# LeoIV/polyaxon

Measured on AMD Instinct MI355X. Metric: HPO trials/hour (whole node) + wall-clock-to-target, ResNet-50 Hyperband sweep, higher is better.
Workload: dtype bf16

## Files before the change

polyaxon_amd/csrc/bn_kernels.hip:

```cpp
#include <hip/hip_runtime.h>

#include "handoff.h"
#include <stdint.h>

#define PLX_API extern "C" __attribute__((visibility("default")))

namespace {

constexpr int kBlock = 256;

struct alignas(16) bf16x8 {
  uint16_t v[8];
};

__device__ __forceinline__ float bf2f(uint16_t b) { return __uint_as_float(((uint32_t)b) << 16); }

__device__ __forceinline__ uint16_t f2bf(float f) {
  return __builtin_bit_cast(uint16_t, (__bf16)f);
}

__device__ __forceinline__ void load8(const bf16x8* p, float* f) {
  const bf16x8 v = *p;
#pragma unroll
  for (int k = 0; k < 8; ++k) f[k] = bf2f(v.v[k]);
// ... 465 lines not shown
        ra[k] += g2;
        rc[k] = fmaf(g2, (x2[k] - mu2[k]) * is2[k], rc[k]);
      }
    }
    float o[8];
#pragma unroll
    for (int k = 0; k < 8; ++k) o[k] = fmaf(A[k], g[k], fmaf(B[k], xv[k], D[k]));
    store8(dx + i, o);
  }
  if constexpr (rp) {
  __shared__ float red[kBlock * 16];
#pragma unroll
  for (int k = 0; k < 8; ++k) {
    red[threadIdx.x * 16 + k] = ra[k];
    red[threadIdx.x * 16 + 8 + k] = rc[k];
  }
  __syncthreads();
  if ((int)threadIdx.x < G) {
    for (int j = 1; j < kBlock / G; ++j) {
      const float* o = red + (j * G + threadIdx.x) * 16;
#pragma unroll
      for (int k = 0; k < 8; ++k) {
        ra[k] += o[k];
        rc[k] += o[8 + k];
      }
    }
    float* pa = rb.part + (int64_t)blockIdx.x * C + cg * 8;
    float* pc = rb.part + ((int64_t)gridDim.x + blockIdx.x) * C + cg * 8;
#pragma unroll
    for (int k = 0; k < 8; ++k) {
      pa[k] = ra[k];
      pc[k] = rc[k];
    }
  }
  }
}

struct Plan {
  int G, Gb, gy, nblk, S;
  int64_t rows_per_block;
};

inline bool plan_for(int64_t M, int C, Plan* p) {
  if (C <= 0 || (C & 7)) return false;
  const int G = C / 8;
  if (G & (G - 1)) return false;
  p->G = G;
  p->Gb = G < kBlock ? G : kBlock;
  p->gy = G / p->Gb;
  const int R = kBlock / p->Gb;
  const int64_t cap = (2048 + p->gy - 1) / p->gy;
  int64_t want = (M + 16 * R - 1) / (16 * R);
  if (want > cap) want = cap;
  if (want < 1) want = 1;
  int64_t rpb = (M + want - 1) / want;
  rpb = (rpb + R - 1) / R * R;
  p->rows_per_block = rpb;
  p->nblk = (int)((M + rpb - 1) / rpb);
  p->S = (p->nblk + kRowsPerSplit - 1) / kRowsPerSplit;
  return true;
}

inline int apply_grid(int64_t n_vec, int G) {
  int64_t g = (n_vec + kBlock - 1) / kBlock;
  if (g > 4096) g = 4096;
  if (g < 1) g = 1;
  const int64_t mult = G > kBlock ? G / kBlock : 1;
  g = (g + mult - 1) / mult * mult;
  return (int)g;
}

inline void launch_dx(hipStream_t stream, int64_t n_vec, int G, const void* x, const uint8_t* mask, const void* dy,
                      void* dx, void* dres, const float* coef, int relu, const ResBn& rb) {
  const dim3 grid(apply_grid(n_vec, G));
  auto k = rb.part == nullptr ? (relu ? bn_bwd_dx_kernel<false, true> : bn_bwd_dx_kernel<false, false>)
           : rb.mask != nullptr ? (relu ? bn_bwd_dx_kernel<true, true, true> : bn_bwd_dx_kernel<true, false, true>)
                                : (relu ? bn_bwd_dx_kernel<true, true> : bn_bwd_dx_kernel<true, false>);
  hipLaunchKernelGGL(k, grid, dim3(kBlock), 0, stream, (const bf16x8*)x, mask, (const bf16x8*)dy, (bf16x8*)dx,
                     (bf16x8*)dres, coef, n_vec, G, relu, rb);
}

inline void launch_apply(hipStream_t stream, int64_t n_vec, int G, const void* x, const void* res, void* y,
                         const float* scale, const float* bias, int relu, uint8_t* mask, const float* rsb) {
  auto k = res != nullptr ? (relu ? bn_apply_kernel<true, true> : bn_apply_kernel<true, false>)
                          : (relu ? bn_apply_kernel<false, true> : bn_apply_kernel<false, false>);
  hipLaunchKernelGGL(k, dim3(apply_grid(n_vec, G)), dim3(kBlock), 0, stream, (const bf16x8*)x, (const bf16x8*)res,
                     (bf16x8*)y, scale, bias, n_vec, G, mask, rsb);
}

inline void reduce_finalize_fwd(hipStream_t stream, const float* part, int nblk, float* l2, unsigned* cnt,
                                const FwdFin& f) {
  const int C = f.C, S = (nblk + kRowsPerSplit - 1) / kRowsPerSplit;
  if (cnt != nullptr) {
    hipLaunchKernelGGL(bn_fwd_reduce_finalize_kernel<kFinNT>, dim3((C + 63) / 64, S), dim3(kFinNT), 0, stream, part, nblk, l2, S,
                       cnt, f);
    return;
  }
  hipLaunchKernelGGL(bn_partial_reduce_kernel<kFinNT>,
                     dim3((C + 63) / 64, S, 2), dim3(kFinNT), 0, stream, part, nblk, C, l2, S);
  hipLaunchKernelGGL(bn_fwd_finalize_kernel<kFinNT>, dim3((C + 63) / 64),
                     dim3(kFinNT), 0, stream, l2, l2 + (int64_t)S * C, S,
                     f.x_row0, C, f.M, f.gamma, f.beta, f.eps, f.momentum, f.running_mean, f.running_var, f.save_mean,
                     f.save_invstd, f.scale, f.bias);
}

inline void reduce_finalize_bwd(hipStream_t stream, const float* part, int nblk, float* l2, unsigned* cnt,
                                const BwdFin& f) {
  const int C = f.C, S = (nblk + kRowsPerSplit - 1) / kRowsPerSplit;
  if (cnt != nullptr) {
    hipLaunchKernelGGL(bn_bwd_reduce_finalize_kernel<kFinNT>, dim3((C + 63) / 64, S), dim3(kFinNT), 0, stream, part, nblk, l2, S,
                       cnt, f);
    return;
  }
  hipLaunchKernelGGL(bn_partial_reduce_kernel<kFinNT>,
                     dim3((C + 63) / 64, S, 2), dim3(kFinNT), 0, stream, part, nblk, C, l2, S);
  hipLaunchKernelGGL(bn_bwd_finalize_kernel<kFinNT>, dim3((C + 63) / 64),
                     dim3(kFinNT), 0, stream, l2, l2 + (int64_t)S * C, S, C,
                     f.M, f.gamma, f.mean, f.invstd, f.dgamma, f.dbeta, f.coef, f.accumulate);
}

struct alignas(8) u8x8 {
  uint8_t v[8];
};

__global__ __launch_bounds__(256) void stem_apply_pool_kernel(const bf16x8* __restrict__ x,
                                                              const float* __restrict__ sb, bf16x8* __restrict__ y,
                                                              u8x8* __restrict__ idx, int N, int H, int W, int G,
                                                              int OH, int OW) {
  const unsigned j = blockIdx.x * 256u + threadIdx.x;
  if (j >= (unsigned)(OW * G)) return;
  const unsigned g = j % (unsigned)G, ow = j / (unsigned)G;
  const int C = G * 8;
  float a[8], b[8];
#pragma unroll
  for (int k = 0; k < 8; ++k) {
    a[k] = sb[g * 8 + k];
    b[k] = sb[C + g * 8 + k];
  }
  for (int row = blockIdx.y; row < N * OH; row += gridDim.y) {
    const int n = row / OH, oh = row - n * OH;
    float best[8];
    uint8_t arg[8];
#pragma unroll
    for (int k = 0; k < 8; ++k) {
      best[k] = -INFINITY;
      arg[k] = 255;
    }
    uint4 q[9];
    bool ok[9];
#pragma unroll
    for (int kh = 0; kh < 3; ++kh) {
      const int ih = oh * 2 - 1 + kh;
      const int ihc = ih < 0 ? 0 : (ih >= H ? H - 1 : ih);
#pragma unroll
      for (int kw = 0; kw < 3; ++kw) {
        const int iw = (int)ow * 2 - 1 + kw;
        const int iwc = iw < 0 ? 0 : (iw >= W ? W - 1 : iw);
        ok[kh * 3 + kw] = ih >= 0 && ih < H && iw >= 0 && iw < W;
        q[kh * 3 + kw] = *(const uint4*)(x + ((size_t)(n * H + ihc) * W + iwc) * G + g);
      }
    }
#pragma unroll
    for (int t9 = 0; t9 < 9; ++t9) {
      const uint32_t qw[4] = {q[t9].x, q[t9].y, q[t9].z, q[t9].w};
#pragma unroll
      for (int k = 0; k < 8; ++k) {
        const float xk = __uint_as_float((k & 1) ? (qw[k >> 1] & 0xffff0000u) : (qw[k >> 1] << 16));
        const float f = (float)(__bf16)fmaxf(fmaf(xk, a[k], b[k]), 0.f);
        if (ok[t9] && (f > best[k] || arg[k] == 255)) {
          best[k] = f;
          arg[k] = (uint8_t)t9;
        }
      }
    }
    bf16x8 o;
    u8x8 m;
#pragma unroll
    for (int k = 0; k < 8; ++k) {
      o.v[k] = f2bf(best[k]);
      m.v[k] = arg[k];
    }
    const size_t t = (size_t)row * OW * G + j;
    y[t] = o;
    idx[t] = m;
  }
}

__device__ __forceinline__ int stem_cover(int i, int O, int* o, int* k) {
  int n = 0;
  if (i & 1) {
    if ((i + 1) >> 1 < O) { o[n] = (i + 1) >> 1; k[n++] = 0; }
    o[n] = (i - 1) >> 1; k[n++] = 2;
  } else if ((i >> 1) < O) {
    o[n] = i >> 1; k[n++] = 1;
  }
  return n;
}

template <bool DX>
__global__ __launch_bounds__(256) void stem_pool_bn_bwd_kernel(const bf16x8* __restrict__ dy, const u8x8* __restrict__ idx,
                                                               const bf16x8* __restrict__ x, const float* __restrict__ sb,
                                                               const float* __restrict__ mean,
                                                               const float* __restrict__ invstd,
                                                               const float* __restrict__ coef, bf16x8* __restrict__ dx,
                                                               float* __restrict__ part, int N, int H, int W, int G,
                                                               int OH, int OW) {
  const int QH = (H + 1) / 2, QW = (W + 1) / 2;
  const unsigned j0 = blockIdx.x * 256u + threadIdx.x;
  const bool active = j0 < (unsigned)(QW * G);
  const unsigned j = active ? j0 : 0u;
  const unsigned g = j % (unsigned)G;
  const int qb = (int)(j / (unsigned)G);
  const int C = G * 8;
  float a[8], b[8], c1[8], c2[8], c3[8], s1[8], s2[8];
#pragma unroll
  for (int k = 0; k < 8; ++k) {
    a[k] = sb[g * 8 + k];
    b[k] = sb[C + g * 8 + k];
    if constexpr (DX) {
      c1[k] = coef[g * 8 + k];
      c2[k] = coef[C + g * 8 + k];
      c3[k] = coef[2 * C + g * 8 + k];
    } else {
      c1[k] = mean[g * 8 + k];
      c2[k] = invstd[g * 8 + k];
      c3[k] = 0.f;
    }
    s1[k] = s2[k] = 0.f;
  }
  for (int row = blockIdx.y; active && row < N * QH; row += gridDim.y) {
    const int n = row / QH, qa = row - n * QH;
    uint2 am[4];
    uint4 d[4], xq[4];
    bool wv[4], pv[4];
#pragma unroll
    for (int p = 0; p < 2; ++p)
#pragma unroll
      for (int q = 0; q < 2; ++q) {
        const int w4 = p * 2 + q, oh = qa + p, ow = qb + q;
        wv[w4] = oh < OH && ow < OW;
        const size_t off = ((size_t)(n * OH + (oh < OH ? oh : OH - 1)) * OW + (ow < OW ? ow : OW - 1)) * G + g;
        am[w4] = *(const uint2*)(idx + off);
        d[w4] = *(const uint4*)(dy + off);
        if (!wv[w4]) am[w4] = make_uint2(0xffffffffu, 0xffffffffu);
        const int ih = 2 * qa + p, iw = 2 * qb + q;
        pv[w4] = ih < H && iw < W;
        xq[w4] = *(const uint4*)(x + ((size_t)(n * H + (ih < H ? ih : H - 1)) * W + (iw < W ? iw : W - 1)) * G + g);
      }
#pragma unroll
    for (int di = 0; di < 2; ++di)
#pragma unroll
      for (int dj = 0; dj < 2; ++dj) {
        const int e = di * 2 + dj;
        const uint32_t xw[4] = {xq[e].x, xq[e].y, xq[e].z, xq[e].w};
        float o[8];
#pragma unroll
        for (int k = 0; k < 8; ++k) {
          float acc = 0.f;
#pragma unroll
          for (int p = 0; p < 2; ++p)
#pragma unroll
            for (int q = 0; q < 2; ++q) {
              const int kh = di + 1 - 2 * p, kw = dj + 1 - 2 * q;
              if (kh < 0 || kw < 0) continue;
              const int w4 = p * 2 + q;
              const uint32_t ab = (k < 4 ? am[w4].x : am[w4].y) >> (8 * (k & 3)) & 0xffu;
              const uint32_t dw = (k >> 1) == 0 ? d[w4].x : (k >> 1) == 1 ? d[w4].y : (k >> 1) == 2 ? d[w4].z : d[w4].w;
              const float dv = __uint_as_float((k & 1) ? (dw & 0xffff0000u) : (dw << 16));
              acc += ab == (uint32_t)(kh * 3 + kw) ? dv : 0.f;
            }
          const float xf = __uint_as_float((k & 1) ? (xw[k >> 1] & 0xffff0000u) : (xw[k >> 1] << 16));
          const float dz = (pv[e] && fmaf(xf, a[k], b[k]) > 0.f) ? (float)(__bf16)acc : 0.f;
          if constexpr (DX) {
            o[k] = fmaf(c1[k], dz, fmaf(c2[k], xf, c3[k]));
          } else {
            s1[k] += dz;
            s2[k] = fmaf(dz, (xf - c1[k]) * c2[k], s2[k]);
          }
        }
        if constexpr (DX) {
          if (pv[e]) store8(dx + ((size_t)(n * H + 2 * qa + di) * W + 2 * qb + dj) * G + g, o);
        }
      }
  }
  if constexpr (!DX) {
    __shared__ float red[256 * 17];
#pragma unroll
    for (int k = 0; k < 8; ++k) {
      red[threadIdx.x * 17 + k] = s1[k];
      red[threadIdx.x * 17 + 8 + k] = s2[k];
    }
    __syncthreads();
    const int nb = gridDim.x * gridDim.y, blk = blockIdx.y * gridDim.x + blockIdx.x;
    for (int e = threadIdx.x; e < G * 16; e += 256) {
      const int gg = e % G, v = e / G;
      float sum = 0.f;
      for (int r = gg; r < 256; r += G) sum += red[r * 17 + v];
      const int c = gg * 8 + (v & 7);
      part[((int64_t)(v < 8 ? 0 : nb) + blk) * C + c] = sum;
    }
  }
}

constexpr int g_stem_bwd_cap = 4096;

inline dim3 stem_bwd_grid(int N, int H, int W, int G, bool dx) {
  const int rows = N * ((H + 1) / 2), cap = dx ? 65535 : g_stem_bwd_cap;
  return dim3((((W + 1) / 2) * G + 255) / 256, rows < cap ? rows : cap);
}

}

PLX_API int64_t plx_bn_workspace(int64_t M, int C) {
  Plan p;
  if (!plan_for(M, C, &p)) return -1;
  return 2 * (int64_t)(p.nblk + p.S) * C;
}

PLX_API int plx_bn_forward(const void* x, const void* res, void* y, int64_t M, int C, const float* gamma,
                           const float* beta, float eps, float momentum, float* running_mean, float* running_var,
                           float* save_mean, float* save_invstd, float* scale_bias ,
                           float* partials , uint8_t* mask ,
                           int relu, const float* res_sb ,
                           unsigned* counters ,
                           hipStream_t stream) {
  Plan p;
  if (!plan_for(M, C, &p) || M < 1) return 1;
  float* psum = partials;
  float* psq = partials + (int64_t)p.nblk * C;
  hipLaunchKernelGGL(bn_stats_kernel, dim3(p.nblk, p.gy), dim3(kBlock), 0, stream, (const bf16x8*)x, M, p.G, p.Gb,
                     p.rows_per_block, psum, psq);
  float* l2 = partials + 2 * (int64_t)p.nblk * C;
  reduce_finalize_fwd(stream, partials, p.nblk, l2, counters,
                      FwdFin{(const uint16_t*)x, C, M, gamma, beta, eps, momentum, running_mean, running_var,
                             save_mean, save_invstd, scale_bias, scale_bias + C});
  const int64_t n_vec = M * p.G;
  if (y != nullptr)
    launch_apply(stream, n_vec, p.G, x, res, y, scale_bias, scale_bias + C, relu, relu ? mask : nullptr, res_sb);
  return (int)hipGetLastError();
}

PLX_API int64_t plx_bn_l2_workspace(int nblk, int C) {
  return 2 * (int64_t)((nblk + kRowsPerSplit - 1) / kRowsPerSplit) * C;
}

PLX_API int plx_bn_forward_from_partials(const void* x, const void* res, void* y, int64_t M, int C,
                                         const float* gamma, const float* beta, float eps, float momentum,
                                         float* running_mean, float* running_var, float* save_mean,
                                         float* save_invstd, float* scale_bias, const float* partials, int nblk,
                                         float* l2, uint8_t* mask, int relu, const float* res_sb,
                                         unsigned* counters, hipStream_t stream) {
  Plan p;
  if (!plan_for(M, C, &p) || M < 1 || nblk < 1) return 1;
  reduce_finalize_fwd(stream, partials, nblk, l2, counters,
                      FwdFin{nullptr, C, M, gamma, beta, eps, momentum, running_mean, running_var, save_mean,
                             save_invstd, scale_bias, scale_bias + C});
  const int64_t n_vec = M * p.G;
  if (y != nullptr)
    launch_apply(stream, n_vec, p.G, x, res, y, scale_bias, scale_bias + C, relu, relu ? mask : nullptr, res_sb);
  return (int)hipGetLastError();
}

PLX_API int plx_bn_apply(const void* x, const void* res, void* y, int64_t M, int C, const float* scale_bias, int relu,
                         hipStream_t stream) {
  Plan p;
  if (!plan_for(M, C, &p)) return 1;
  const int64_t n_vec = M * p.G;
  launch_apply(stream, n_vec, p.G, x, res, y, scale_bias, scale_bias + C, relu, nullptr, nullptr);
  return (int)hipGetLastError();
}

PLX_API int plx_bn_apply_res_relu(const void* x, const void* res, void* y, int64_t M, int C, const float* scale_bias,
                                  uint8_t* mask, const float* res_sb, hipStream_t stream) {
  Plan p;
  if (!plan_for(M, C, &p) || M < 1 || res == nullptr || mask == nullptr) return 1;
  launch_apply(stream, M * p.G, p.G, x, res, y, scale_bias, scale_bias + C, 1, mask, res_sb);
  return (int)hipGetLastError();
}

PLX_API int plx_bn_dx_blocks(int64_t M, int C) {
  Plan p;
  if (!plan_for(M, C, &p)) return -1;
  return apply_grid(M * p.G, p.G);
}

PLX_API int plx_bn_backward(const void* x, const uint8_t* mask, const void* dy, void* dx, void* dres, int64_t M, int C,
                            const float* gamma, const float* save_mean, const float* save_invstd, float* dgamma,
                            float* dbeta, float* coef , float* partials , int relu,
                            int accumulate, const ResBn* resbn , unsigned* counters,
                            hipStream_t stream) {
  Plan p;
  if (!plan_for(M, C, &p) || M < 1 || (relu && mask == nullptr)) return 1;
  if (resbn != nullptr && (dres == nullptr || resbn->part == nullptr)) return 1;
  const ResBn rb = resbn != nullptr ? *resbn : ResBn{};
  float* pa = partials;
  float* pb = partials + (int64_t)p.nblk * C;
  hipLaunchKernelGGL(relu ? bn_bwd_reduce_kernel<true> : bn_bwd_reduce_kernel<false>, dim3(p.nblk, p.gy), dim3(kBlock), 0, stream, (const bf16x8*)x,
                     mask, (const bf16x8*)dy, M, p.G, p.Gb, p.rows_per_block, save_mean, save_invstd,
                     relu, pa, pb);
  float* l2 = partials + 2 * (int64_t)p.nblk * C;
  reduce_finalize_bwd(stream, partials, p.nblk, l2, counters,
                      BwdFin{C, M, gamma, save_mean, save_invstd, dgamma, dbeta, coef, accumulate});
  const int64_t n_vec = M * p.G;
  launch_dx(stream, n_vec, p.G, x, mask, dy, dx, dres, coef, relu, rb);
  return (int)hipGetLastError();
}

PLX_API int plx_bn_backward_from_partials(const void* x, const uint8_t* mask, const void* dy, void* dx, void* dres,
                                          int64_t M, int C, const float* gamma, const float* save_mean,
                                          const float* save_invstd, float* dgamma, float* dbeta, float* coef,
                                          const float* partials, int nblk, float* l2, int relu, int accumulate,
                                          const ResBn* resbn, unsigned* counters, hipStream_t stream) {
  Plan p;
  if (!plan_for(M, C, &p) || M < 1 || nblk < 1 || (relu && mask == nullptr)) return 1;
  if (resbn != nullptr && (dres == nullptr || resbn->part == nullptr)) return 1;
  const ResBn rb = resbn != nullptr ? *resbn : ResBn{};
  reduce_finalize_bwd(stream, partials, nblk, l2, counters,
                      BwdFin{C, M, gamma, save_mean, save_invstd, dgamma, dbeta, coef, accumulate});
  const int64_t n_vec = M * p.G;
  launch_dx(stream, n_vec, p.G, x, mask, dy, dx, dres, coef, relu, rb);
  return (int)hipGetLastError();
}

PLX_API int plx_bn_backward_coef(const void* x, const uint8_t* mask, const void* dy, int64_t M, int C,
                                 const float* gamma, const float* save_mean, const float* save_invstd, float* dgamma,
                                 float* dbeta, float* coef, float* partials, int relu, int accumulate,
                                 unsigned* counters, hipStream_t stream) {
  Plan p;
  if (!plan_for(M, C, &p) || M < 1 || (relu && mask == nullptr)) return 1;
  float* pa = partials;
  float* pb = partials + (int64_t)p.nblk * C;
  hipLaunchKernelGGL(relu ? bn_bwd_reduce_kernel<true> : bn_bwd_reduce_kernel<false>, dim3(p.nblk, p.gy), dim3(kBlock), 0, stream, (const bf16x8*)x,
                     mask, (const bf16x8*)dy, M, p.G, p.Gb, p.rows_per_block, save_mean, save_invstd,
                     relu, pa, pb);
  reduce_finalize_bwd(stream, partials, p.nblk, partials + 2 * (int64_t)p.nblk * C, counters,
                      BwdFin{C, M, gamma, save_mean, save_invstd, dgamma, dbeta, coef, accumulate});
  return (int)hipGetLastError();
}

PLX_API int plx_bn_backward_coef_from_partials(int64_t M, int C, const float* gamma, const float* save_mean,
                                               const float* save_invstd, float* dgamma, float* dbeta, float* coef,
                                               const float* partials, int nblk, float* l2, int accumulate,
                                               unsigned* counters, hipStream_t stream) {
  Plan p;
  if (!plan_for(M, C, &p) || M < 1 || nblk < 1) return 1;
  reduce_finalize_bwd(stream, partials, nblk, l2, counters,
                      BwdFin{C, M, gamma, save_mean, save_invstd, dgamma, dbeta, coef, accumulate});
  return (int)hipGetLastError();
}

PLX_API int plx_stem_bn_pool_forward(const void* x, void* y, void* idx, int N, int H, int W, int C, const float* gamma,
                                     const float* beta, float eps, float momentum, float* running_mean,
                                     float* running_var, float* save_mean, float* save_invstd, float* scale_bias,
                                     float* partials, const float* ext_part, int ext_nblk, unsigned* counters,
                                     hipStream_t stream) {
  const int G = C / 8;
  if (N <= 0 || H <= 0 || W <= 0 || C % 8 || G > 256 || 256 % G) return 1;
  const int rc = ext_part != nullptr
                     ? plx_bn_forward_from_partials(x, nullptr, nullptr, (int64_t)N * H * W, C, gamma, beta, eps,
                                                    momentum, running_mean, running_var, save_mean, save_invstd,
                                                    scale_bias, ext_part, ext_nblk, partials, nullptr, 1, nullptr,
                                                    counters, stream)
                     : plx_bn_forward(x, nullptr, nullptr, (int64_t)N * H * W, C, gamma, beta, eps, momentum,
                                      running_mean, running_var, save_mean, save_invstd, scale_bias, partials, nullptr,
                                      1, nullptr, counters, stream);
  if (rc) return rc;
  const int OH = (H - 1) / 2 + 1, OW = (W - 1) / 2 + 1;
  const int rows = N * OH;
  hipLaunchKernelGGL(stem_apply_pool_kernel, dim3((OW * G + 255) / 256, rows < 65535 ? rows : 65535), dim3(256), 0,
                     stream, (const bf16x8*)x, scale_bias, (bf16x8*)y, (u8x8*)idx, N, H, W, G, OH, OW);
  return (int)hipGetLastError();
}


PLX_API int64_t plx_stem_bn_pool_bwd_workspace(int N, int H, int W, int C) {
  const dim3 g = stem_bwd_grid(N, H, W, C / 8, false);
  const int64_t nblk = (int64_t)g.x * g.y;
  return 2 * (nblk + (nblk + kRowsPerSplit - 1) / kRowsPerSplit) * C;
}

PLX_API int plx_stem_bn_pool_backward(const void* dy, const void* idx, const void* x, void* dx, int N, int H, int W,
                                      int C, const float* gamma, const float* save_mean, const float* save_invstd,
                                      const float* scale_bias, float* dgamma, float* dbeta, float* coef,
                                      float* workspace, int accumulate, unsigned* counters, hipStream_t stream) {
  const int G = C / 8;
  if (N <= 0 || H <= 0 || W <= 0 || C % 8 || G > 256 || 256 % G) return 1;
  const int OH = (H - 1) / 2 + 1, OW = (W - 1) / 2 + 1;
  const dim3 grid = stem_bwd_grid(N, H, W, G, false), grid_dx = stem_bwd_grid(N, H, W, G, true);
  const int nblk = grid.x * grid.y;
  hipLaunchKernelGGL(stem_pool_bn_bwd_kernel<false>, grid, dim3(256), 0, stream, (const bf16x8*)dy, (const u8x8*)idx,
                     (const bf16x8*)x, scale_bias, save_mean, save_invstd, (const float*)nullptr, (bf16x8*)nullptr,
                     workspace, N, H, W, G, OH, OW);
  reduce_finalize_bwd(stream, workspace, nblk, workspace + 2 * (int64_t)nblk * C, counters,
                      BwdFin{C, (int64_t)N * H * W, gamma, save_mean, save_invstd, dgamma, dbeta, coef, accumulate});
  hipLaunchKernelGGL(stem_pool_bn_bwd_kernel<true>, grid_dx, dim3(256), 0, stream, (const bf16x8*)dy, (const u8x8*)idx,
                     (const bf16x8*)x, scale_bias, save_mean, save_invstd, coef, (bf16x8*)dx, (float*)nullptr, N, H,
                     W, G, OH, OW);
  return (int)hipGetLastError();
}
```

polyaxon_amd/ops/_native.py:

```python
from __future__ import annotations

import ctypes
import hashlib
import os
import shutil
import subprocess
import threading
from pathlib import Path
from typing import Dict, Iterable, List, Optional

PKG_DIR = Path(__file__).resolve().parent.parent
CSRC = PKG_DIR / "csrc"
OUT = PKG_DIR / "_native"
ARCH = os.environ.get("PLX_OFFLOAD_ARCH", "gfx950")
ROCM = Path(os.environ.get("ROCM_PATH", "/opt/rocm"))

LIBRARIES: Dict[str, dict] = {
    "plx_train": {"sources": ["train_kernels.hip"], "kind": "hip", "link": []},
    "plx_polytune": {"sources": ["polytune_kernels.hip"], "kind": "hip", "link": []},
    "plx_bn": {"sources": ["bn_kernels.hip"], "kind": "hip", "link": []},
    "plx_procmon": {"sources": ["procmon.cpp"], "kind": "cpp", "link": ["-lpthread"]},
    "plx_gp": {"sources": ["gp_kernels.hip", "gp_chol.hip"], "kind": "hip", "link": []},
    "plx_rms": {"sources": ["rmsnorm.hip"], "kind": "hip", "link": []},
    "plx_conv": {"sources": ["conv_gemm.hip"], "kind": "hip", "link": []},
    "plx_pool": {"sources": ["pool_kernels.hip"], "kind": "hip", "link": []},
    "plx_lm": {"sources": ["lm_kernels.hip"], "kind": "hip", "link": []},
    "plx_gemm": {"sources": ["gemm256.hip"], "kind": "hip", "link": []},
    "plx_attn": {"sources": ["attn_kernels.hip"], "kind": "hip", "link": []},
    "plx_rccl": {"sources": ["rccl_comm.cpp"], "kind": "hip_host", "link": ["-lrccl", "-pthread"]},
}

_lock = threading.Lock()
_loaded: Dict[str, ctypes.CDLL] = {}


def _register(name: str, sources: List[str], kind: str, link: Optional[List[str]] = None) -> None:
    LIBRARIES[name] = {"sources": sources, "kind": kind, "link": list(link or [])}


def lib_path(name: str) -> Path:
    return OUT / f"lib{name}.so"


def _digest(sources: Iterable[Path], flags: List[str]) -> str:
    h = hashlib.sha256()
    for s in sources:
        h.update(s.read_bytes())
    for hdr in sorted(CSRC.glob("*.h")):
        h.update(hdr.read_bytes())
    h.update(" ".join(flags).encode())
    return h.hexdigest()[:16]


def _flags(kind: str) -> List[str]:
    common = ["-O3", "-std=c++17", "-shared", "-fPIC", "-Wall", "-Wno-unused-function", f"-I{CSRC}"]
    if kind == "hip":
        fences = ["-DPLX_HANDOFF_FENCES=1"] if os.environ.get("PLX_HANDOFF_FENCES") == "1" else []
        return common + [f"--offload-arch={ARCH}", "-munsafe-fp-atomics"] + fences
    if kind == "hip_host":
        return common + [f"-I{ROCM / 'include'}", "-D__HIP_PLATFORM_AMD__"]
    return common


def build(name: str, force: bool = False, verbose: bool = False) -> Path:
    spec = LIBRARIES[name]
    srcs = [CSRC / s for s in spec["sources"]]
    flags = _flags(spec["kind"])
    out = lib_path(name)
    stamp = out.with_suffix(".so.sha")
    digest = _digest(srcs, flags + spec["link"])
    if not force and out.exists() and stamp.exists() and stamp.read_text().strip() == digest:
        return out
    OUT.mkdir(parents=True, exist_ok=True)
    if spec["kind"] in ("hip", "hip_host"):
        cc = shutil.which("hipcc") or str(ROCM / "bin" / "hipcc")
    else:
        cc = shutil.which("g++") or "g++"
    link = list(spec["link"])
    if spec["kind"] == "hip_host":
        link = [f"-L{ROCM / 'lib'}", f"-Wl,-rpath,{ROCM / 'lib'}"] + link + ["-lamdhip64"]
    tmp = out.with_suffix(f".so.tmp{os.getpid()}")
    cmd = [cc, *flags, *map(str, srcs), "-o", str(tmp), *link]
    if verbose:
        print(" ".join(cmd))
    proc = subprocess.run(cmd, capture_output=True, text=True)
    if proc.returncode != 0:
        raise RuntimeError(f"native build of {name} failed:\n{' '.join(cmd)}\n{proc.stderr[-6000:]}")
    os.replace(tmp, out)
    stamp.write_text(digest)
    return out


def _stale(name: str) -> bool:
    spec = LIBRARIES[name]
    stamp = lib_path(name).with_suffix(".so.sha")
    if not stamp.exists():
        return False
    try:
        digest = _digest([CSRC / s for s in spec["sources"]], _flags(spec["kind"]) + spec["link"])
    except OSError:
        return False
    return stamp.read_text().strip() != digest


def build_all(force: bool = False, verbose: bool = False) -> List[Path]:
    return [build(n, force=force, verbose=verbose) for n in LIBRARIES]


def available(name: str) -> bool:
    return lib_path(name).exists()


_SIZES: Dict[tuple, int] = {}


_COUNTERS: Dict[tuple, object] = {}


def capturing() -> bool:
    import torch

    return torch.cuda.is_available() and torch.cuda.is_current_stream_capturing()


def cached(cache: dict, key, make, ok=None):
    v = cache.get(key)
    if v is not None and (ok is None or ok(v)):
        return v
    v = make()
    if not capturing():
        cache[key] = v
    return v


def counters(device, key: str, n: int = 4096):
    import torch

    return cached(_COUNTERS, (str(device), key), lambda: torch.zeros(n, dtype=torch.int32, device=device))


def current_stream() -> int:
    import torch

    return torch._C._cuda_getCurrentRawStream(torch._C._cuda_getDevice())


def size(libname: str, fn: str, *args: int) -> int:
    key = (fn,) + args
    v = _SIZES.get(key)
    if v is None:
        v = _SIZES[key] = int(getattr(lib(libname), fn)(*args))
    return v


def lib(name: str) -> ctypes.CDLL:
    with _lock:
        if name in _loaded:
            return _loaded[name]
        path = lib_path(name)
        if not path.exists() or os.environ.get("PLX_NATIVE_REBUILD") == "1" or _stale(name):
            build(name, force=os.environ.get("PLX_NATIVE_REBUILD") == "1")
        handle = ctypes.CDLL(str(path), mode=ctypes.RTLD_GLOBAL)
        _declare(name, handle)
        if name == "plx_conv" and os.environ.get("PLX_WGRAD_ATOMIC"):
            handle.plx_set_tn_atomic(int(os.environ["PLX_WGRAD_ATOMIC"]))
        if name == "plx_gemm" and os.environ.get("PLX_GEMM_WAVES"):
            handle.plx_gemm256_set_waves(int(os.environ["PLX_GEMM_WAVES"]))
        _loaded[name] = handle
        return handle


_P = ctypes.c_void_p
_I = ctypes.c_int
_L = ctypes.c_int64
_U64 = ctypes.c_uint64
_F = ctypes.c_float
_D = ctypes.c_double

SIGNATURES: Dict[str, Dict[str, list]] = {
    "plx_train": {
        "plx_sgd_flat": [_P, _P, _P, _L, _L, _P, _P, _P],
        "plx_adamw_flat": [_P, _P, _P, _P, _L, _L, _P, _P, _P],
        "plx_adamw_mixed": [_P, _P, _P, _P, _P, _L, _I, _P, _P, _P],
        "plx_sgd_flat_clip": [_P, _P, _P, _L, _L, _P, _P, _P, _P],
        "plx_adamw_flat_clip": [_P, _P, _P, _P, _L, _L, _P, _P, _P, _P],
        "plx_adamw_mixed_clip": [_P, _P, _P, _P, _P, _L, _I, _P, _P, _P, _P],
        "plx_gradnorm_blocks": [_L],
        "plx_gradnorm_partials": [_P, _I, _L, _P, _P],
        "plx_gradnorm_finalize": [_P, _I, _P, _P, _P],
        "plx_lr_schedule": [_P, _P, _P, _P],
        "plx_cast_lp": [_P, _P, _L, _P],
        "plx_init_flat": [_P, _P, _P, _P, _I, _P, _P, _U64, _P],
        "plx_zero_flat": [_P, _L, _P],
        "plx_record_metric": [_P, _I, _P, _P, _I, _P],
        "plx_commit_metric": [_P, _P, _I, _I, _P, _I, _P],
        "plx_synth_images": [_P, _P, _I, _I, _I, _P, _I, _I, _F, _U64, _P, _P],
        "plx_set_adamw_grid_cap": [_I],
        "plx_set_adamw_wide": [_I],
    },
    "plx_bn": {
        "plx_bn_workspace": [_L, _I],
        "plx_bn_forward": [_P, _P, _P, _L, _I, _P, _P, _F, _F, _P, _P, _P, _P, _P, _P, _P, _I, _P, _P, _P],
        "plx_bn_apply": [_P, _P, _P, _L, _I, _P, _I, _P],
        "plx_bn_apply_res_relu": [_P, _P, _P, _L, _I, _P, _P, _P, _P],
        "plx_bn_l2_workspace": [_I, _I],
        "plx_bn_forward_from_partials": [_P, _P, _P, _L, _I, _P, _P, _F, _F, _P, _P, _P, _P, _P, _P, _I, _P, _P,
                                         _I, _P, _P, _P],
        "plx_bn_backward": [_P, _P, _P, _P, _P, _L, _I, _P, _P, _P, _P, _P, _P, _P, _I, _I, _P, _P, _P],
        "plx_bn_dx_blocks": [_L, _I],
        "plx_bn_backward_from_partials": [_P, _P, _P, _P, _P, _L, _I, _P, _P, _P, _P, _P, _P, _P, _I, _P, _I, _I, _P,
                                          _P, _P],
        "plx_bn_backward_coef": [_P, _P, _P, _L, _I, _P, _P, _P, _P, _P, _P, _P, _I, _I, _P, _P],
        "plx_bn_backward_coef_from_partials": [_L, _I, _P, _P, _P, _P, _P, _P, _P, _I, _P, _I, _P, _P],
        "plx_stem_bn_pool_forward": [_P, _P, _P, _I, _I, _I, _I, _P, _P, _F, _F, _P, _P, _P, _P, _P, _P, _P, _I, _P,
                                     _P],
        "plx_stem_bn_pool_bwd_workspace": [_I, _I, _I, _I],
        "plx_stem_bn_pool_backward": [_P, _P, _P, _P, _I, _I, _I, _I, _P, _P, _P, _P, _P, _P, _P, _P, _I, _P, _P],
    },
    "plx_procmon": {
        "plx_pm_create": [],
        "plx_pm_destroy": [_P],
        "plx_pm_spawn": [_P, _P, _P, ctypes.c_char_p, ctypes.c_char_p, ctypes.POINTER(_I)],
        "plx_pm_wait": [_P, _I, ctypes.POINTER(_I), ctypes.POINTER(_I)],
        "plx_pm_wake": [_P],
        "plx_pm_signal": [_P, _I, _I, _I],
        "plx_pm_count": [_P],
    },
    "plx_gp": {
        "plx_gp_kmat": [_P, _P, _I, _I, _I, _P, _I, _I, _F, _F, _F, _I, _F, _P, _P, _D, _I, _P],
        "plx_gp_chol": [_P, _I, _I, _P, _P],
        "plx_gp_kmat_batch_f64": [_P, _I, _I, _P, _I, _P, _I, _L, _I, _D, _D, _D, _P, _P, _D, _I, _P],
        "plx_gp_matern_table": [_D, _D, _D, _I, _P, _P, _P],
        "plx_gp_chol_aug_f64": [_P, _I, _I, _I, _L, _I, _P, _P, _P],
        "plx_gp_chol_scratch_doubles": [],
        "plx_gp_lml_f64": [_P, _I, _I, _L, _I, _P, _P, _P],
        "plx_gp_acq_rows": [_P, _I, _I, _P, _F, _I, _F, _F, _F, _P, _P, _P, _P],
        "plx_gp_predict_acq": [_P, _I, _P, _I, _I, _P, _I, _P, _I, _F, _F, _F, _F, _I, _F, _F, _F, _P, _P, _P, _P,
                               _P, _P, _P, _D, _I, _P],
        "plx_gp_ascent": [_P, _P, _I, _P, _P, _P, _I, _I, _P, _P, _I, _F, _F, _F, _F, _I, _F, _F, _F, _I, _P, _P, _D, _I,
                          _P],
    },
    "plx_conv": {
        "plx_gemm_nt": [_P, _P, _P, _I, _I, _I, _I, _I, _I, _P, _P, _P, _I, _P, _P, _P],
        "plx_gemm_nt_bndx": [_P, _P, _P, _P, _P, _P, _P, _I, _I, _I, _I, _I, _P, _I, _P, _P, _P],
        "plx_gemm_nt_bnapply": [_P, _P, _P, _P, _P, _P, _P, _P, _I, _I, _I, _I, _I, _P, _P],
        "plx_gemm_nt_rows_per_block": [_I],
        "plx_gemm_tn_workspace": [_I, _I, _I, _I],
        "plx_set_tn_v2": [_I, _I],
        "plx_set_tn2_stem": [_I],
        "plx_set_tn2_c64": [_I],
        "plx_set_tn_atomic": [_I],
        "plx_tn_plan_slices": [_I, _I, _I, _I, _I],
        "plx_gemm_tn": [_P, _P, _P, _P, _I, _I, _I, _I, _I, _I, _P, _I, _I, _P],
        "plx_weight_prep": [_P, _P, _P, _I, _I, _P],
        "plx_weight_prepk": [_P, _L, _L, _L, _L, _P, _P, _I, _I, _I, _P],
        "plx_weight_prep_all": [_P, _P, _P, _P, _I, _I, _P],
        "plx_stem_pack_input": [_P, _P, _I, _I, _I, _P],
        "plx_stem_pack_weight": [_P, _L, _L, _L, _L, _P, _I, _P],
        "plx_stem_conv_rows_per_block": [],
        "plx_stem_conv_fwd": [_P, _P, _P, _I, _I, _I, _P, _P, _P],
        "plx_stem_conv_wgrad_workspace": [_I, _I, _I, _I],
        "plx_stem_conv_wgrad": [_P, _P, _P, _L, _L, _L, _L, _P, _I, _I, _I, _P, _I, _I, _P],
        "plx_conv_fwd": [_P, _P, _P, _I, _I, _I, _I, _I, _I, _I, _P, _P, _P],
        "plx_conv_dgrad": [_P, _P, _P, _I, _I, _I, _I, _I, _I, _I, _P, _P, _P, _P],
        "plx_conv_dgrad_blocks": [_I, _I, _I, _I, _I, _I, _I],
        "plx_conv_wgrad_workspace": [_I, _I, _I, _I, _I, _I, _I, _I],
        "plx_conv_wgrad": [_P, _P, _P, _P, _I, _I, _I, _I, _I, _I, _I, _P, _I, _I, _P],
    },
    "plx_lm": {
        "plx_qkv_rope_fwd": [_P, _P, _P, _P, _P, _P, _L, _I, _I, _I, _I, _I, _P],
        "plx_qkv_rope_bwd": [_P, _P, _P, _P, _P, _P, _L, _I, _I, _I, _I, _I, _P],
        "plx_swiglu_fwd": [_P, _P, _L, _I, _P],
        "plx_swiglu_bwd": [_P, _P, _P, _L, _I, _P],
        "plx_xent_fwd": [_P, _P, _P, _P, _I, _I, _I, _P],
        "plx_xent_bwd": [_P, _P, _P, _P, _P, _I, _I, _I, _P],
        "plx_xent_cls_fwd": [_P, _P, _P, _P, _I, _I, _P],
        "plx_xent_cls_bwd": [_P, _P, _P, _P, _P, _I, _I, _F, _P],
        "plx_colsum_splits": [_L, _I],
        "plx_colsum": [_P, _L, _I, _P, _P, _P, _I, _P],
        "plx_gelu_bwd_colsum": [_P, _P, _P, _L, _I, _P, _P, _P, _I, _P],
    },
    "plx_gemm": {
        "plx_gemm256": [_P, _P, _P, _P, _I, _I, _I, _I, _I, _I, _I, _I, _F, _I, _P],
        "plx_gemm256_bias": [_P, _P, _P, _P, _I, _I, _I, _I, _I, _I, _I, _I, _F, _I, _P, _P],
        "plx_gemm256_ex": [_P, _P, _P, _P, _I, _I, _I, _I, _I, _I, _I, _I, _F, _I, _P, _P, _P],
        "plx_gemm256_exv": [_P, _P, _P, _P, _I, _I, _I, _I, _I, _I, _I, _I, _F, _I, _P, _P, _I, _P],
        "plx_gemm256_splits": [_I, _I, _I],
        "plx_gemm256_set_split_target": [_I],
        "plx_gemm256_set_waves": [_I],
        "plx_gemm256_set_group": [_I],
        "plx_gemm256_tile": [],
        "plx_gemm256_sk_ws": [_I, _I, _I],
        "plx_gemm256_sk_plan": [_I, _I, _I, ctypes.POINTER(_I), ctypes.POINTER(_I)],
        "plx_gemm256_set_sk_force": [_I],
        "plx_gemm256_sk": [_P, _P, _P, _P, _P, _I, _I, _I, _I, _I, _I, _I, _I, _F, _P, _P, _P, _P],
    },
    "plx_attn": {
        "plx_attn_fwd": [_P, _I, _P],
        "plx_attn_bwd": [_P, _I, _P, _P],
        "plx_attn_bwd_workspace": [_I, _I, _I, _I, _I],
        "plx_attn_args_size": [],
        "plx_attn_set_fwd_waves": [_I],
        "plx_attn_set_dq_waves": [_I],
        "plx_attn_set_dkdv_waves": [_I],
    },
    "plx_pool": {
        "plx_maxpool3s2_forward": [_P, _P, _P, _I, _I, _I, _I, _P],
        "plx_gap_forward": [_P, _P, _I, _I, _I, _P],
        "plx_gap_backward": [_P, _P, _I, _I, _I, _P],
        "plx_maxpool3s2_backward": [_P, _P, _P, _I, _I, _I, _I, _P],
    },
    "plx_rms": {
        "plx_rms_forward": [_P, _P, _P, _P, _L, _I, _F, _P],
        "plx_rms_bwd_blocks": [_L],
        "plx_ln_bwd_blocks": [_L, _I],
        "plx_add_ln_forward": [_P, _P, _P, _P, _P, _P, _P, _P, _L, _I, _F, _P],
        "plx_add_rms_forward": [_P, _P, _P, _P, _P, _P, _L, _I, _F, _P],
        "plx_add_rms_backward": [_P, _P, _P, _P, _P, _P, _P, _L, _I, _P],
        "plx_add_ln_backward": [_P, _P, _P, _P, _P, _P, _P, _P, _P, _L, _I, _P],
        "plx_partial_colsum_workspace": [_I, _I, _I],
        "plx_partial_colsum": [_P, _P, _I, _I, _I, _P, _P, _P, _P, _I, _I, _P],
        "plx_rms_backward": [_P, _P, _P, _P, _P, _P, _L, _I, _P],
        "plx_ln_forward": [_P, _P, _P, _P, _P, _P, _L, _I, _F, _P],
        "plx_ln_backward": [_P, _P, _P, _P, _P, _P, _P, _P, _L, _I, _P],
    },
    "plx_rccl": {
        "plx_rccl_unique_id": [ctypes.c_char_p],
        "plx_rccl_init": [ctypes.c_char_p, _I, _I, _I, _L, _L, ctypes.POINTER(_I)],
        "plx_rccl_all_reduce": [_P, _P, _P, _L, _I, _I, _P],
        "plx_rccl_all_gather": [_P, _P, _P, _L, _I, _P],
        "plx_rccl_reduce_scatter": [_P, _P, _P, _L, _I, _I, _P],
        "plx_rccl_broadcast": [_P, _P, _P, _L, _I, _I, _P],
        "plx_rccl_bus_bw": [_P, _P, _L, _I, _P, ctypes.POINTER(_D), ctypes.POINTER(_D)],
        "plx_rccl_destroy": [_P],
        "plx_rccl_status": [_P],
        "plx_rccl_pending": [_P],
        "plx_rccl_set_timeout": [_P, _L],
        "plx_rccl_abort": [_P],
        "plx_rccl_error": [_I],
    },
    "plx_polytune": {
        "plx_topk_brackets": [_P, _P, _I, _I, _I, _I, _P, _P],
        "plx_philox_sample": [_P, _P, _I, _L, _L, ctypes.c_uint64, _P, _P],
        "plx_philox_desc_size": [],
        "plx_early_stop_any": [_P, _I, _I, _P, _P, _P, _I, _P, _P],
    },
}


RESTYPES: Dict[str, object] = {"plx_attn_bwd_workspace": ctypes.c_longlong, "plx_conv_wgrad_workspace": _L, "plx_bn_workspace": _L, "plx_bn_l2_workspace": _L, "plx_partial_colsum_workspace": _L, "plx_stem_bn_pool_bwd_workspace": _L, "plx_gemm_tn_workspace": _L, "plx_gemm256_sk_ws": ctypes.c_longlong, "plx_stem_conv_wgrad_workspace": _L, "plx_pm_create": _P, "plx_pm_destroy": None, "plx_set_tn_v2": None, "plx_set_tn2_stem": None, "plx_set_tn2_c64": None, "plx_set_tn_atomic": None, "plx_set_adamw_grid_cap": None, "plx_set_adamw_wide": None, "plx_attn_set_fwd_waves": None, "plx_attn_set_dq_waves": None, "plx_attn_set_dkdv_waves": None, "plx_gemm256_set_split_target": None,
                               "plx_pm_wake": None, "plx_rccl_init": _P, "plx_rccl_error": ctypes.c_char_p}


def _declare(name: str, handle: ctypes.CDLL) -> None:
    for fn, argtypes in SIGNATURES.get(name, {}).items():
        f = getattr(handle, fn)
        f.argtypes = argtypes
        f.restype = RESTYPES.get(fn, _I)


class ResBnArgs(ctypes.Structure):
    _fields_ = [("x", _P), ("mask", _P), ("mean", _P), ("invstd", _P), ("part", _P)]


class BnBwdArgs(ctypes.Structure):
    _fields_ = [("x", _P), ("mask", _P), ("mean", _P), ("invstd", _P), ("part", _P), ("part_ld", _I),
                ("blk_off", _I), ("skip_h", _I), ("skip_w", _I)]


def check(rc: int, what: str) -> None:
    if rc != 0:
        raise RuntimeError(f"{what} failed with code {rc}")
```

Measured before the change: 12700.

## Add thin stem BN+maxpool kernels with row-strip reuse and LDS-staged constants

Adds new forward and backward kernels for the stem BN+ReLU+maxpool path, enabled by default through a global flag. The forward kernel walks a strip of output rows per thread and carries the transformed boundary input row into the next output row, so overlapping 3x3 window rows are not reloaded or recomputed. The backward kernels stage per-channel constants in LDS and process 2x2 input quads from the pooled indices, with scheduling fences to control register pressure. The dx pass also tiles several rows per block. This is meant to cut redundant loads and ALU work in a memory-bound stage, at the cost of more complex code and possible register pressure or occupancy loss.

```diff
diff --git a/polyaxon_amd/csrc/bn_kernels.hip b/polyaxon_amd/csrc/bn_kernels.hip
--- a/polyaxon_amd/csrc/bn_kernels.hip
+++ b/polyaxon_amd/csrc/bn_kernels.hip
@@ -791,6 +791,259 @@
   }
 }
 
+int g_bn_thin = 1;
+
+__device__ __forceinline__ int thin_slot(int arr, int k, int grp, int ngrp) {
+  return ((arr * 2 + (k >> 2)) * ngrp + grp) * 4 + (k & 3);
+}
+
+__device__ __forceinline__ void thin_trip_fence() { asm volatile("" ::: "memory"); }
+
+__device__ __forceinline__ void thin_pin4(uint32_t& a, uint32_t& b, uint32_t& c, uint32_t& d) {
+  asm volatile("" : "+v"(a), "+v"(b), "+v"(c), "+v"(d));
+}
+
+__device__ __forceinline__ void thin_sched_fence() { __builtin_amdgcn_sched_barrier(0); }
+
+constexpr int kStemFwdRows = 8;
+constexpr int kStemDxRows = 4;
+
+__device__ __forceinline__ uint4 stem_tf(const uint4 q, const float* a, const float* b) {
+  const uint32_t qw[4] = {q.x, q.y, q.z, q.w};
+  uint32_t r[4];
+#pragma unroll
+  for (int w = 0; w < 4; ++w) {
+    const float lo = fmaxf(fmaf(__uint_as_float(qw[w] << 16), a[2 * w], b[2 * w]), 0.f);
+    const float hi = fmaxf(fmaf(__uint_as_float(qw[w] & 0xffff0000u), a[2 * w + 1], b[2 * w + 1]), 0.f);
+    r[w] = (uint32_t)f2bf(lo) | ((uint32_t)f2bf(hi) << 16);
+  }
+  return make_uint4(r[0], r[1], r[2], r[3]);
+}
+
+__device__ __forceinline__ void stem_tap(const uint4 f4, bool ok, bool& none, uint32_t t9, float* best, uint32_t* arg) {
+  const uint32_t fw[4] = {f4.x, f4.y, f4.z, f4.w};
+#pragma unroll
+  for (int k = 0; k < 8; ++k) {
+    const float f = __uint_as_float((k & 1) ? (fw[k >> 1] & 0xffff0000u) : (fw[k >> 1] << 16));
+    if (ok && (f > best[k] || none)) {
+      best[k] = f;
+      arg[k] = t9;
+    }
+  }
+  none = none && !ok;
+  thin_sched_fence();
+}
+
+__global__ __launch_bounds__(256) void stem_apply_pool_thin_kernel(const bf16x8* __restrict__ x,
+                                                                   const float* __restrict__ sb,
+                                                                   bf16x8* __restrict__ y, u8x8* __restrict__ idx,
+                                                                   int H, int W, int G, int OH, int OW, int gx,
+                                                                   int cpi) {
+  const unsigned bx = blockIdx.x % (unsigned)gx, chunk = blockIdx.x / (unsigned)gx;
+  const unsigned j = bx * 256u + threadIdx.x;
+  if (j >= (unsigned)(OW * G)) return;
+  const unsigned g = j % (unsigned)G, ow = j / (unsigned)G;
+  const int C = G * 8;
+  float a[8], b[8];
+#pragma unroll
+  for (int k = 0; k < 8; ++k) {
+    a[k] = sb[g * 8 + k];
+    b[k] = sb[C + g * 8 + k];
+  }
+  const int n = (int)chunk / cpi, oh0 = ((int)chunk - n * cpi) * kStemFwdRows;
+  const int oh1 = oh0 + kStemFwdRows < OH ? oh0 + kStemFwdRows : OH;
+  int col[3];
+  bool cok[3];
+#pragma unroll
+  for (int kw = 0; kw < 3; ++kw) {
+    const int iw = (int)ow * 2 - 1 + kw;
+    cok[kw] = iw >= 0 && iw < W;
+    col[kw] = (iw < 0 ? 0 : (iw >= W ? W - 1 : iw)) * G;
+  }
+  const bf16x8* xn = x + (size_t)n * H * W * G + g;
+  uint4 pr[3], q[6];
+  {
+    const int ihp = oh0 > 0 ? 2 * oh0 - 1 : 0, ihb = 2 * oh0 + 1 < H ? 2 * oh0 + 1 : H - 1;
+#pragma unroll
+    for (int kw = 0; kw < 3; ++kw) {
+      pr[kw] = *(const uint4*)(xn + (size_t)ihp * W * G + col[kw]);
+      q[kw] = *(const uint4*)(xn + (size_t)(2 * oh0) * W * G + col[kw]);
+      q[3 + kw] = *(const uint4*)(xn + (size_t)ihb * W * G + col[kw]);
+    }
+#pragma unroll
+    for (int kw = 0; kw < 3; ++kw) pr[kw] = stem_tf(pr[kw], a, b);
+  }
+  for (int oh = oh0; oh < oh1; ++oh) {
+    uint4 nq[6];
+    {
+      const int ohn = oh + 1 < oh1 ? oh + 1 : oh, ihb = 2 * ohn + 1 < H ? 2 * ohn + 1 : H - 1;
+#pragma unroll
+      for (int kw = 0; kw < 3; ++kw) {
+        nq[kw] = *(const uint4*)(xn + (size_t)(2 * ohn) * W * G + col[kw]);
+        nq[3 + kw] = *(const uint4*)(xn + (size_t)ihb * W * G + col[kw]);
+      }
+    }
+    float best[8];
+    uint32_t arg[8];
+#pragma unroll
+    for (int k = 0; k < 8; ++k) {
+      best[k] = -INFINITY;
+      arg[k] = 255;
+    }
+    bool none = true;
+    const bool r0 = oh > 0, r2 = 2 * oh + 1 < H;
+#pragma unroll
+    for (int kw = 0; kw < 3; ++kw) stem_tap(pr[kw], r0 && cok[kw], none, kw, best, arg);
+#pragma unroll
+    for (int kw = 0; kw < 3; ++kw) stem_tap(stem_tf(q[kw], a, b), cok[kw], none, 3 + kw, best, arg);
+#pragma unroll
+    for (int kw = 0; kw < 3; ++kw) {
+      pr[kw] = stem_tf(q[3 + kw], a, b);
+      stem_tap(pr[kw], r2 && cok[kw], none, 6 + kw, best, arg);
+    }
+    bf16x8 o;
+    u8x8 m;
+#pragma unroll
+    for (int k = 0; k < 8; ++k) {
+      o.v[k] = f2bf(best[k]);
+      m.v[k] = (uint8_t)arg[k];
+    }
+    const size_t t = (size_t)(n * OH + oh) * OW * G + j;
+    y[t] = o;
+    idx[t] = m;
+#pragma unroll
+    for (int e = 0; e < 6; ++e) q[e] = nq[e];
+  }
+}
+
+template <bool DX>
+__global__ __launch_bounds__(256) void stem_pool_bn_bwd_thin_kernel(
+    const bf16x8* __restrict__ dy, const u8x8* __restrict__ idx, const bf16x8* __restrict__ x,
+    const float* __restrict__ sb, const float* __restrict__ mean, const float* __restrict__ invstd,
+    const float* __restrict__ coef, bf16x8* __restrict__ dx, float* __restrict__ part, int N, int H, int W, int G,
+    int OH, int OW) {
+  extern __shared__ float4 thin_lds[];
+  constexpr int NA = DX ? 5 : 4;
+  const int QH = (H + 1) / 2, QW = (W + 1) / 2;
+  const unsigned j0 = blockIdx.x * 256u + threadIdx.x;
+  const bool active = j0 < (unsigned)(QW * G);
+  const unsigned j = active ? j0 : 0u;
+  const unsigned g = j % (unsigned)G;
+  const int qb = (int)(j / (unsigned)G);
+  const int C = G * 8;
+  for (int e = threadIdx.x; e < NA * C; e += 256) {
+    const int arr = e / C, c = e - arr * C;
+    const float* src = arr == 0 ? sb : arr == 1 ? sb + C : DX ? coef + (arr - 2) * C : arr == 2 ? mean : invstd;
+    ((float*)thin_lds)[thin_slot(arr, c & 7, c >> 3, G)] = src[c];
+  }
+  __syncthreads();
+  float s1[8], s2[8];
+#pragma unroll
+  for (int k = 0; k < 8; ++k) s1[k] = s2[k] = 0.f;
+  const int rows = N * QH;
+  const int row0 = DX ? blockIdx.y * kStemDxRows : blockIdx.y, step = DX ? 1 : gridDim.y;
+  const int row1 = DX ? (row0 + kStemDxRows < rows ? row0 + kStemDxRows : rows) : rows;
+  for (int row = row0; active && row < row1; row += step) {
+    thin_trip_fence();
+    const int n = row / QH, qa = row - n * QH;
+    uint2 am[4];
+    uint4 d[4], xq[4];
+    bool pv[4];
+#pragma unroll
+    for (int p = 0; p < 2; ++p)
+#pragma unroll
+      for (int q = 0; q < 2; ++q) {
+        const int w4 = p * 2 + q, oh = qa + p, ow = qb + q;
+        const size_t off = ((size_t)(n * OH + (oh < OH ? oh : OH - 1)) * OW + (ow < OW ? ow : OW - 1)) * G + g;
+        am[w4] = *(const uint2*)(idx + off);
+        d[w4] = *(const uint4*)(dy + off);
+        if (!(oh < OH && ow < OW)) am[w4] = make_uint2(0xffffffffu, 0xffffffffu);
+        const int ih = 2 * qa + p, iw = 2 * qb + q;
+        pv[w4] = ih < H && iw < W;
+        xq[w4] = *(const uint4*)(x + ((size_t)(n * H + (ih < H ? ih : H - 1)) * W + (iw < W ? iw : W - 1)) * G + g);
+      }
+    uint32_t amw[4][2], dw[4][4], xw[4][4];
+#pragma unroll
+    for (int w4 = 0; w4 < 4; ++w4) {
+      amw[w4][0] = am[w4].x, amw[w4][1] = am[w4].y;
+      dw[w4][0] = d[w4].x, dw[w4][1] = d[w4].y, dw[w4][2] = d[w4].z, dw[w4][3] = d[w4].w;
+      xw[w4][0] = xq[w4].x, xw[w4][1] = xq[w4].y, xw[w4][2] = xq[w4].z, xw[w4][3] = xq[w4].w;
+    }
+    uint32_t ow4[4][4];
+#pragma unroll
+    for (int h = 0; h < 2; ++h) {
+      float cst[NA][4];
+#pragma unroll
+      for (int arr = 0; arr < NA; ++arr) {
+        const float4 v = thin_lds[(arr * 2 + h) * G + g];
+        cst[arr][0] = v.x, cst[arr][1] = v.y, cst[arr][2] = v.z, cst[arr][3] = v.w;
+      }
+      thin_pin4(amw[0][h], amw[1][h], amw[2][h], amw[3][h]);
+#pragma unroll
+      for (int kp = 0; kp < 2; ++kp) {
+        const int w = h * 2 + kp;
+        thin_pin4(dw[0][w], dw[1][w], dw[2][w], dw[3][w]);
+        thin_pin4(xw[0][w], xw[1][w], xw[2][w], xw[3][w]);
+#pragma unroll
+        for (int k2 = 0; k2 < 2; ++k2) {
+          const int kk = kp * 2 + k2, k = h * 4 + kk;
+#pragma unroll
+          for (int e = 0; e < 4; ++e) {
+            const int di = e >> 1, dj = e & 1;
+            float acc = 0.f;
+#pragma unroll
+            for (int p = 0; p < 2; ++p)
+#pragma unroll
+              for (int q = 0; q < 2; ++q) {
+                const int kh = di + 1 - 2 * p, kw = dj + 1 - 2 * q;
+                if (kh < 0 || kw < 0) continue;
+                const int w4 = p * 2 + q;
+                const uint32_t ab = amw[w4][h] >> (8 * kk) & 0xffu;
+                const float dv = __uint_as_float(k2 ? (dw[w4][w] & 0xffff0000u) : (dw[w4][w] << 16));
+                acc += ab == (uint32_t)(kh * 3 + kw) ? dv : 0.f;
+              }
+            const float xf = __uint_as_float(k2 ? (xw[e][w] & 0xffff0000u) : (xw[e][w] << 16));
+            const float dz = (pv[e] && fmaf(xf, cst[0][kk], cst[1][kk]) > 0.f) ? (float)(__bf16)acc : 0.f;
+            if constexpr (DX) {
+              const uint32_t ob = f2bf(fmaf(cst[2][kk], dz, fmaf(cst[3][kk], xf, cst[NA - 1][kk])));
+              ow4[e][w] = k2 ? (ow4[e][w] | (ob << 16)) : ob;
+            } else {
+              s1[k] += dz;
+              s2[k] = fmaf(dz, (xf - cst[2][kk]) * cst[3][kk], s2[k]);
+            }
+          }
+        }
+        if constexpr (DX) thin_pin4(ow4[0][w], ow4[1][w], ow4[2][w], ow4[3][w]);
+        thin_sched_fence();
+      }
+    }
+    if constexpr (DX) {
+#pragma unroll
+      for (int e = 0; e < 4; ++e)
+        if (pv[e])
+          *(uint4*)(dx + ((size_t)(n * H + 2 * qa + (e >> 1)) * W + 2 * qb + (e & 1)) * G + g) =
+              make_uint4(ow4[e][0], ow4[e][1], ow4[e][2], ow4[e][3]);
+    }
+  }
+  if constexpr (!DX) {
+    __shared__ float red[256 * 17];
+#pragma unroll
+    for (int k = 0; k < 8; ++k) {
+      red[threadIdx.x * 17 + k] = s1[k];
+      red[threadIdx.x * 17 + 8 + k] = s2[k];
+    }
+    __syncthreads();
+    const int nb = gridDim.x * gridDim.y, blk = blockIdx.y * gridDim.x + blockIdx.x;
+    for (int e = threadIdx.x; e < G * 16; e += 256) {
+      const int gg = e % G, v = e / G;
+      float sum = 0.f;
+      for (int r = gg; r < 256; r += G) sum += red[r * 17 + v];
+      const int c = gg * 8 + (v & 7);
+      part[((int64_t)(v < 8 ? 0 : nb) + blk) * C + c] = sum;
+    }
+  }
+}
+
 constexpr int g_stem_bwd_cap = 4096;
 
 inline dim3 stem_bwd_grid(int N, int H, int W, int G, bool dx) {
@@ -799,6 +1052,8 @@
 }
 
 }
+
+PLX_API void plx_bn_set_thin(int on) { g_bn_thin = on != 0; }
 
 PLX_API int64_t plx_bn_workspace(int64_t M, int C) {
   Plan p;
@@ -956,6 +1211,13 @@
   if (rc) return rc;
   const int OH = (H - 1) / 2 + 1, OW = (W - 1) / 2 + 1;
   const int rows = N * OH;
+  if (g_bn_thin) {
+    const int gx = (OW * G + 255) / 256, cpi = (OH + kStemFwdRows - 1) / kStemFwdRows;
+    if ((int64_t)gx * N * cpi > 0x7fffffff) return 1;
+    hipLaunchKernelGGL(stem_apply_pool_thin_kernel, dim3(gx * N * cpi), dim3(256), 0, stream, (const bf16x8*)x,
+                       scale_bias, (bf16x8*)y, (u8x8*)idx, H, W, G, OH, OW, gx, cpi);
+    return (int)hipGetLastError();
+  }
   hipLaunchKernelGGL(stem_apply_pool_kernel, dim3((OW * G + 255) / 256, rows < 65535 ? rows : 65535), dim3(256), 0,
                      stream, (const bf16x8*)x, scale_bias, (bf16x8*)y, (u8x8*)idx, N, H, W, G, OH, OW);
   return (int)hipGetLastError();
@@ -977,6 +1239,24 @@
   const int OH = (H - 1) / 2 + 1, OW = (W - 1) / 2 + 1;
   const dim3 grid = stem_bwd_grid(N, H, W, G, false), grid_dx = stem_bwd_grid(N, H, W, G, true);
   const int nblk = grid.x * grid.y;
+  if (g_bn_thin) {
+    const int rows = N * ((H + 1) / 2);
+    const dim3 grid_thin(grid.x, (rows + kStemDxRows - 1) / kStemDxRows);
+    hipLaunchKernelGGL(stem_pool_bn_bwd_thin_kernel<false>, grid, dim3(256), sizeof(float) * 4 * C, stream,
+                       (const bf16x8*)dy, (const u8x8*)idx, (const bf16x8*)x, scale_bias, save_mean, save_invstd,
+                       (const float*)nullptr, (bf16x8*)nullptr, workspace, N, H, W, G, OH, OW);
+    reduce_finalize_bwd(stream, workspace, nblk, workspace + 2 * (int64_t)nblk * C, counters,
+                        BwdFin{C, (int64_t)N * H * W, gamma, save_mean, save_invstd, dgamma, dbeta, coef, accumulate});
+    if (grid_thin.y <= 65535)
+      hipLaunchKernelGGL(stem_pool_bn_bwd_thin_kernel<true>, grid_thin, dim3(256), sizeof(float) * 5 * C, stream,
+                         (const bf16x8*)dy, (const u8x8*)idx, (const bf16x8*)x, scale_bias, save_mean, save_invstd,
+                         coef, (bf16x8*)dx, (float*)nullptr, N, H, W, G, OH, OW);
+    else
+      hipLaunchKernelGGL(stem_pool_bn_bwd_kernel<true>, grid_dx, dim3(256), 0, stream, (const bf16x8*)dy,
+                         (const u8x8*)idx, (const bf16x8*)x, scale_bias, save_mean, save_invstd, coef, (bf16x8*)dx,
+                         (float*)nullptr, N, H, W, G, OH, OW);
+    return (int)hipGetLastError();
+  }
   hipLaunchKernelGGL(stem_pool_bn_bwd_kernel<false>, grid, dim3(256), 0, stream, (const bf16x8*)dy, (const u8x8*)idx,
                      (const bf16x8*)x, scale_bias, save_mean, save_invstd, (const float*)nullptr, (bf16x8*)nullptr,
                      workspace, N, H, W, G, OH, OW);
diff --git a/polyaxon_amd/ops/_native.py b/polyaxon_amd/ops/_native.py
--- a/polyaxon_amd/ops/_native.py
+++ b/polyaxon_amd/ops/_native.py
@@ -164,6 +164,8 @@
         _declare(name, handle)
         if name == "plx_conv" and os.environ.get("PLX_WGRAD_ATOMIC"):
             handle.plx_set_tn_atomic(int(os.environ["PLX_WGRAD_ATOMIC"]))
+        if name == "plx_bn" and os.environ.get("PLX_BN_THIN"):
+            handle.plx_bn_set_thin(int(os.environ["PLX_BN_THIN"]))
         if name == "plx_gemm" and os.environ.get("PLX_GEMM_WAVES"):
             handle.plx_gemm256_set_waves(int(os.environ["PLX_GEMM_WAVES"]))
         _loaded[name] = handle
@@ -199,6 +201,7 @@
         "plx_set_adamw_wide": [_I],
     },
     "plx_bn": {
+        "plx_bn_set_thin": [_I],
         "plx_bn_workspace": [_L, _I],
         "plx_bn_forward": [_P, _P, _P, _L, _I, _P, _P, _F, _F, _P, _P, _P, _P, _P, _P, _P, _I, _P, _P, _P],
         "plx_bn_apply": [_P, _P, _P, _L, _I, _P, _I, _P],
@@ -348,7 +351,7 @@
 }
 
 
-RESTYPES: Dict[str, object] = {"plx_attn_bwd_workspace": ctypes.c_longlong, "plx_conv_wgrad_workspace": _L, "plx_bn_workspace": _L, "plx_bn_l2_workspace": _L, "plx_partial_colsum_workspace": _L, "plx_stem_bn_pool_bwd_workspace": _L, "plx_gemm_tn_workspace": _L, "plx_gemm256_sk_ws": ctypes.c_longlong, "plx_stem_conv_wgrad_workspace": _L, "plx_pm_create": _P, "plx_pm_destroy": None, "plx_set_tn_v2": None, "plx_set_tn2_stem": None, "plx_set_tn2_c64": None, "plx_set_tn_atomic": None, "plx_set_adamw_grid_cap": None, "plx_set_adamw_wide": None, "plx_attn_set_fwd_waves": None, "plx_attn_set_dq_waves": None, "plx_attn_set_dkdv_waves": None, "plx_gemm256_set_split_target": None,
+RESTYPES: Dict[str, object] = {"plx_attn_bwd_workspace": ctypes.c_longlong, "plx_conv_wgrad_workspace": _L, "plx_bn_workspace": _L, "plx_bn_l2_workspace": _L, "plx_partial_colsum_workspace": _L, "plx_stem_bn_pool_bwd_workspace": _L, "plx_gemm_tn_workspace": _L, "plx_gemm256_sk_ws": ctypes.c_longlong, "plx_stem_conv_wgrad_workspace": _L, "plx_pm_create": _P, "plx_pm_destroy": None, "plx_set_tn_v2": None, "plx_set_tn2_stem": None, "plx_set_tn2_c64": None, "plx_set_tn_atomic": None, "plx_bn_set_thin": None, "plx_set_adamw_grid_cap": None, "plx_set_adamw_wide": None, "plx_attn_set_fwd_waves": None, "plx_attn_set_dq_waves": None, "plx_attn_set_dkdv_waves": None, "plx_gemm256_set_split_target": None,
                                "plx_pm_wake": None, "plx_rccl_init": _P, "plx_rccl_error": ctypes.c_char_p}
 
 
```

Measured after the change: 12840, median of 6. 1.01x the previous value.
